# prs-eth/ResDepth

Hardware: AMD Instinct MI355X
Metric: DSM tiles/sec fwd+bwd (256x256, 3-ch, depth-5 U-Net) (higher is better)
Workload: dtype f32

## Files before the change

### resdepth_amd/csrc/rd_wgrad_strip.hip

```cpp
#include <stdlib.h>

#include "rd_common.h"
#include "rd_mfma_dev.h"

namespace rd {

struct WsParams {
    const float* dz;
    const float* x;
    float* slab;
    int Cin, Cout, M, N;
    int H, W;
    int strips_x, chunks_y, rows_per_chunk, reps;
    int tiles_ci, tiles_mn;
    unsigned a_bytes, b_bytes;
    const unsigned* a_amax;
    const unsigned* b_amax;
    int n_img;
};

typedef short v4s16 __attribute__((ext_vector_type(4)));
template <typename FR>
__device__ __forceinline__ FR lds_tr2(const float* smem_base, int byte_off, int second) {
    typedef __attribute__((address_space(3))) v4s16* lds_p;
    const char* b = reinterpret_cast<const char*>(smem_base) + byte_off;
    const v4s16 lo = __builtin_amdgcn_ds_read_tr16_b64_v4i16((lds_p)(b));
    const v4s16 hi = __builtin_amdgcn_ds_read_tr16_b64_v4i16((lds_p)(b + second));
    typedef short v8s16 __attribute__((ext_vector_type(8)));
    const v8s16 r = {lo.x, lo.y, lo.z, lo.w, hi.x, hi.y, hi.z, hi.w};
    return __builtin_bit_cast(FR, r);
}

template <int NP, int NCO, int NCI, bool W8>
__device__ __forceinline__ void wgrad_strip_tr_body(const WsParams& p, float* smem, const Quant qz) {
    typedef typename frag_of<NP>::type FR;
    constexpr int NT = NP == 3 ? 2 : 3;
    static_assert(NCO * NCI == 4, "four waves");
    constexpr int TA = 64 * NCO, TB = 64 * NCI;
    constexpr int APX = 3 * TA + (NCO == 4 ? 64 : NCO == 2 ? 64 : 0), BPX = 3 * TB + (NCI == 2 ? 64 : 0);
    static_assert((APX / 4) % 64 == 16 || (APX / 4) % 64 == 48, "dz pixel stride");
    static_assert((BPX / 4) % 64 == 16 || (BPX / 4) % 64 == 48, "x pixel stride");
    constexpr int HPX = W8 ? 20 : 18;
    constexpr int ASTAGE = 16 * APX, BSLOT = HPX * BPX;
    constexpr int RINGB = 2 * ASTAGE;
    constexpr int AQ = 8 * NCO, BQ = 8 * NCI;
    constexpr int AI = 16 * AQ / 256, BI = (HPX * BQ + 255) / 256;

    const int gb = xcd_remap(blockIdx.x, gridDim.x);
    const int split = gb / p.tiles_mn;
    const int lb = gb - split * p.tiles_mn;
    const int tile_ci = lb % p.tiles_ci, tile_m = lb / p.tiles_ci;
    const int m0 = tile_m * (32 * NCO), ci0 = tile_ci * (32 * NCI);
    int img = 0, x0 = 0, ya = 0, yb = 0;
    const int H = p.H, W = p.W;
    const int t = threadIdx.x, lane = t & 63, wave = t >> 6;
    const int cw = wave / NCI, cb = wave % NCI;

    int a_wr[AI], b_wr[BI];
    int a_px[AI], a_ch[AI], b_hp[BI], b_ch[BI];
    bool b_act[BI];
#pragma unroll
    for (int k = 0; k < AI; ++k) {
        const int e = t + 256 * k, cq = e % AQ, px = e / AQ;
        a_px[k] = px;
        a_ch[k] = m0 + cq * 4 < p.Cout ? m0 + cq * 4 : -1;
        a_wr[k] = px * APX + cq * 8;
    }
#pragma unroll
    for (int k = 0; k < BI; ++k) {
        const int e = t + 256 * k, cq = e % BQ, hp = e / BQ;
        b_act[k] = e < HPX * BQ;
        b_hp[k] = hp;
        b_ch[k] = (b_act[k] && ci0 + cq * 4 < p.Cin) ? ci0 + cq * 4 : -1;
        b_wr[k] = hp * BPX + cq * 8;
    }
    const __amdgpu_buffer_rsrc_t rsA = make_rsrc(p.dz, p.a_bytes), rsB = make_rsrc(p.x, p.b_bytes);
    const unsigned rowA = (unsigned)W * p.Cout * 4, rowB = (unsigned)W * p.Cin * 4;
    unsigned baseA = 0, baseB = 0, voffA[AI], voffB[BI];
    auto set_strip = [&](int sid) {
        const int sx = sid % p.strips_x;
        const int cy = (sid / p.strips_x) % p.chunks_y;
        img = sid / (p.strips_x * p.chunks_y);
        x0 = sx * 16;
        ya = cy * p.rows_per_chunk;
        yb = ya + p.rows_per_chunk;
        if (W8) img *= 2;
        baseA = (unsigned)img * H * rowA;
        baseB = (unsigned)img * H * rowB;
        if (W8) {
            const bool two = img + 1 < p.n_img;
#pragma unroll
            for (int k = 0; k < AI; ++k) {
                const int sub = a_px[k] >> 3, xx = a_px[k] & 7;
                voffA[k] = (a_ch[k] >= 0 && (sub == 0 || two)) ? (unsigned)(((sub * 64 + xx) * p.Cout + a_ch[k]) * 4) : kOOB;
            }
#pragma unroll
            for (int k = 0; k < BI; ++k) {
                const int sub = b_hp[k] >= 10 ? 1 : 0, px = b_hp[k] - 10 * sub - 1;
                voffB[k] = (b_ch[k] >= 0 && (unsigned)px < 8u && (sub == 0 || two)) ? (unsigned)(((sub * 64 + px) * p.Cin + b_ch[k]) * 4) : kOOB;
            }
            return;
        }
#pragma unroll
        for (int k = 0; k < AI; ++k) voffA[k] = a_ch[k] >= 0 ? (unsigned)(((x0 + a_px[k]) * p.Cout + a_ch[k]) * 4) : kOOB;
#pragma unroll
        for (int k = 0; k < BI; ++k) {
            const int px = x0 - 1 + b_hp[k];
            voffB[k] = (b_ch[k] >= 0 && (unsigned)px < (unsigned)W) ? (unsigned)((px * p.Cin + b_ch[k]) * 4) : kOOB;
        }
    };
    auto load_task = [&](int yy, float4 (&v)[AI + BI]) {
        const int ra = yy + 1, rb = yy + 2;
        const bool oka = ra >= ya && ra < yb, okb = rb >= 0 && rb < H && rb <= yb;
        const unsigned sa = (unsigned)__builtin_amdgcn_readfirstlane(oka ? (int)(baseA + (unsigned)ra * rowA) : 0);
        const unsigned sb = (unsigned)__builtin_amdgcn_readfirstlane(okb ? (int)(baseB + (unsigned)rb * rowB) : 0);
#pragma unroll
        for (int k = 0; k < AI; ++k) v[k] = buf_load4(rsA, oka ? voffA[k] : kOOB, sa);
#pragma unroll
        for (int k = 0; k < BI; ++k) v[AI + k] = buf_load4(rsB, okb ? voffB[k] : kOOB, sb);
    };
    auto put = [&](char* dst, int tstride, const float4 x, float qs) {
        uint2 ph, pm, pl;
        split_pack4v<NP, false>(x.x, x.y, x.z, x.w, qs, ph, pm, pl);
        *reinterpret_cast<uint2*>(dst) = ph;
        *reinterpret_cast<uint2*>(dst + tstride) = pm;
        if (kterm3<NP>()) *reinterpret_cast<uint2*>(dst + 2 * tstride) = pl;
    };
    auto store_task = [&](int yy, const float4 (&v)[AI + BI]) {
        char* sa = reinterpret_cast<char*>(smem) + ((yy + 1) & 1) * ASTAGE;
#pragma unroll
        for (int k = 0; k < AI; ++k) put(sa + a_wr[k], TA, v[k], qz.sa);
        char* sb = reinterpret_cast<char*>(smem) + RINGB + ((yy + 3) & 3) * BSLOT;
#pragma unroll
        for (int k = 0; k < BI; ++k)
            if (b_act[k]) put(sb + b_wr[k], TB, v[AI + k], qz.sb);
    };

    const int li = lane & 15, lg = lane >> 4, nb = lg & 1, hk = lg >> 1;
    const int a_rd = (8 * hk + (li >> 2)) * APX + (32 * cw + 16 * nb + 4 * (li & 3)) * 2;
    const int b_rd = (8 * hk + (li >> 2) + (W8 ? 2 * hk : 0)) * BPX + (32 * cb + 16 * nb + 4 * (li & 3)) * 2;
    const int lrow = lane & 31, half = lane >> 5;

    f32x16 acc[9];
#pragma unroll
    for (int tp = 0; tp < 9; ++tp)
#pragma unroll
        for (int r = 0; r < 16; ++r) acc[tp][r] = 0.f;

    constexpr int PA[6] = {2, 1, 0, 1, 0, 0}, PB[6] = {0, 1, 2, 0, 1, 0};
    auto mma_row = [&](int y) {
        const int a_stage = (y & 1) * ASTAGE;
        FR af[3], bf[2][3][3];
        auto read_b = [&](int dy, FR (&dst)[3][3]) {
            const int slot = RINGB + ((y + dy) & 3) * BSLOT;
#pragma unroll
            for (int d = 0; d < 3; ++d)
#pragma unroll
                for (int q = 0; q < NT; ++q) dst[d][q] = lds_tr2<FR>(smem, slot + b_rd + d * BPX + q * TB, 4 * BPX);
        };
#pragma unroll
        for (int q = 0; q < NT; ++q) af[q] = lds_tr2<FR>(smem, a_stage + a_rd + q * TA, 4 * APX);
        read_b(0, bf[0]);
#pragma unroll
        for (int dy = 0; dy < 3; ++dy) {
            if (dy < 2) read_b(dy + 1, bf[(dy + 1) & 1]);
#if RD_WG_FENCE
            if constexpr (NP == 3) __builtin_amdgcn_sched_barrier(0);
#endif
#pragma unroll
            for (int t6 = lo0<NP>(); t6 < 6; ++t6)
#pragma unroll
                for (int d = 0; d < 3; ++d) acc[dy * 3 + d] = mfma16<NP>(af[PA[t6]], bf[dy & 1][d][PB[t6]], acc[dy * 3 + d]);
        }
    };

    float4 v0[AI + BI], v1[AI + BI];
    for (int rep = 0; rep < p.reps; ++rep) {
        set_strip(split * p.reps + rep);
        const int ys = ya - 3;
        load_task(ys, v0);
        load_task(ys + 1, v1);
        store_task(ys, v0);
        load_task(ys + 2, v0);
        __syncthreads();
        store_task(ys + 1, v1);
        load_task(ys + 3, v1);
        __syncthreads();
        store_task(ys + 2, v0);
        load_task(ys + 4, v0);
        __syncthreads();
        for (int yy = ya; yy < yb; yy += 2) {
            store_task(yy, v1);
            load_task(yy + 2, v1);
            mma_row(yy);
            __syncthreads();
            store_task(yy + 1, v0);
            load_task(yy + 3, v0);
            mma_row(yy + 1);
            __syncthreads();
        }
    }

    float* out = p.slab + (long)split * p.M * p.N;
    const int cwu = __builtin_amdgcn_readfirstlane(cw), cbu = __builtin_amdgcn_readfirstlane(cb);
    if (m0 + 32 * NCO <= p.M && (long)(32 * NCO) * p.N * 4 < 0x7fffffffL) {
        const __amdgpu_buffer_rsrc_t rsO = make_rsrc(out + (long)m0 * p.N + ci0, (unsigned)((long)(32 * NCO) * p.N * 4));
        const unsigned lane_off = (unsigned)(((4 * half) * p.N + lrow) * 4);
        const int rowN = __builtin_amdgcn_readfirstlane(p.N * 4);
        const int base = (cwu * 32) * rowN + cbu * 128;
#pragma unroll
        for (int tp = 0; tp < 9; ++tp) {
            const int tapo = base + tp * p.Cin * 4;
#pragma unroll
            for (int r = 0; r < 16; ++r)
                __builtin_amdgcn_raw_buffer_store_b32(__float_as_int(scale_q<NP>(acc[tp][r], qz.dexp)), rsO, lane_off, (unsigned)(tapo + ((r & 3) + 8 * (r >> 2)) * rowN), 0);
        }
        return;
    }
#pragma unroll
    for (int tp = 0; tp < 9; ++tp) {
        const int n = tp * p.Cin + ci0 + cb * 32 + lrow;
#pragma unroll
        for (int r = 0; r < 16; ++r) {
            const int m = m0 + cw * 32 + (r & 3) + 8 * (r >> 2) + 4 * half;
            if (m < p.M) out[(long)m * p.N + n] = scale_q<NP>(acc[tp][r], qz.dexp);
        }
    }
}

template <int NCO, int NCI, bool W8>
__device__ __forceinline__ void wgrad_strip_rot_body(const WsParams& p, float* smem, const Quant qz) {
    typedef f16x8 FR;
    static_assert(NCO * NCI == 4, "four waves");
    constexpr int TA = 64 * NCO, TB = 64 * NCI;
    constexpr int APX = 3 * TA + (NCO == 4 ? 64 : NCO == 2 ? 64 : 0), BPX = 3 * TB + (NCI == 2 ? 64 : 0);
    constexpr int HPX = W8 ? 20 : 18;
    constexpr int ASTAGE = 16 * APX, BSLOT = HPX * BPX;
    constexpr int RINGB = 4 * ASTAGE;
    constexpr int AQ = 8 * NCO, BQ = 8 * NCI;
    constexpr int AI = 16 * AQ / 256, BI = (HPX * BQ + 255) / 256;

    const int gb = xcd_remap(blockIdx.x, gridDim.x);
    const int split = gb / p.tiles_mn;
    const int lb = gb - split * p.tiles_mn;
    const int tile_ci = lb % p.tiles_ci, tile_m = lb / p.tiles_ci;
    const int m0 = tile_m * (32 * NCO), ci0 = tile_ci * (32 * NCI);
    int img = 0, x0 = 0, ya = 0, yb = 0;
    const int H = p.H, W = p.W;
    const int t = threadIdx.x, lane = t & 63, wave = t >> 6;
    const int cw = wave / NCI, cb = wave % NCI;

    int a_wr[AI], b_wr[BI];
    int a_px[AI], a_ch[AI], b_hp[BI], b_ch[BI];
    bool b_act[BI];
#pragma unroll
    for (int k = 0; k < AI; ++k) {
        const int e = t + 256 * k, cq = e % AQ, px = e / AQ;
        a_px[k] = px;
        a_ch[k] = m0 + cq * 4 < p.Cout ? m0 + cq * 4 : -1;
        a_wr[k] = px * APX + cq * 8;
    }
#pragma unroll
    for (int k = 0; k < BI; ++k) {
        const int e = t + 256 * k, cq = e % BQ, hp = e / BQ;
        b_act[k] = e < HPX * BQ;
        b_hp[k] = hp;
        b_ch[k] = (b_act[k] && ci0 + cq * 4 < p.Cin) ? ci0 + cq * 4 : -1;
        b_wr[k] = hp * BPX + cq * 8;
    }
    const __amdgpu_buffer_rsrc_t rsA = make_rsrc(p.dz, p.a_bytes), rsB = make_rsrc(p.x, p.b_bytes);
    const unsigned rowA = (unsigned)W * p.Cout * 4, rowB = (unsigned)W * p.Cin * 4;
    unsigned baseA = 0, baseB = 0, voffA[AI], voffB[BI];
    auto set_strip = [&](int sid) {
        const int sx = sid % p.strips_x;
        const int cy = (sid / p.strips_x) % p.chunks_y;
        img = sid / (p.strips_x * p.chunks_y);
        x0 = sx * 16;
        ya = cy * p.rows_per_chunk;
        yb = ya + p.rows_per_chunk;
        if (W8) img *= 2;
        baseA = (unsigned)img * H * rowA;
        baseB = (unsigned)img * H * rowB;
        if (W8) {
            const bool two = img + 1 < p.n_img;
#pragma unroll
            for (int k = 0; k < AI; ++k) {
                const int sub = a_px[k] >> 3, xx = a_px[k] & 7;
                voffA[k] = (a_ch[k] >= 0 && (sub == 0 || two)) ? (unsigned)(((sub * 64 + xx) * p.Cout + a_ch[k]) * 4) : kOOB;
            }
#pragma unroll
            for (int k = 0; k < BI; ++k) {
                const int sub = b_hp[k] >= 10 ? 1 : 0, px = b_hp[k] - 10 * sub - 1;
                voffB[k] = (b_ch[k] >= 0 && (unsigned)px < 8u && (sub == 0 || two)) ? (unsigned)(((sub * 64 + px) * p.Cin + b_ch[k]) * 4) : kOOB;
            }
            return;
        }
#pragma unroll
        for (int k = 0; k < AI; ++k) voffA[k] = a_ch[k] >= 0 ? (unsigned)(((x0 + a_px[k]) * p.Cout + a_ch[k]) * 4) : kOOB;
#pragma unroll
        for (int k = 0; k < BI; ++k) {
            const int px = x0 - 1 + b_hp[k];
            voffB[k] = (b_ch[k] >= 0 && (unsigned)px < (unsigned)W) ? (unsigned)((px * p.Cin + b_ch[k]) * 4) : kOOB;
        }
    };
    auto load_task = [&](int k, float4 (&v)[AI + BI]) {
        const int r = k + 2;
        const bool oka = r >= ya && r < yb, okb = r >= 0 && r < H && r <= yb;
        const unsigned sa = (unsigned)__builtin_amdgcn_readfirstlane(oka ? (int)(baseA + (unsigned)r * rowA) : 0);
        const unsigned sb = (unsigned)__builtin_amdgcn_readfirstlane(okb ? (int)(baseB + (unsigned)r * rowB) : 0);
#pragma unroll
        for (int i = 0; i < AI; ++i) v[i] = buf_load4(rsA, oka ? voffA[i] : kOOB, sa);
#pragma unroll
        for (int i = 0; i < BI; ++i) v[AI + i] = buf_load4(rsB, okb ? voffB[i] : kOOB, sb);
    };
    auto put = [&](char* dst, int tstride, const float4 x, float qs) {
        uint2 ph, pm, pl;
        split_pack4v<3, false>(x.x, x.y, x.z, x.w, qs, ph, pm, pl);
        *reinterpret_cast<uint2*>(dst) = ph;
        *reinterpret_cast<uint2*>(dst + tstride) = pm;
    };
    auto store_task = [&](int k, const float4 (&v)[AI + BI]) {
        char* sa = reinterpret_cast<char*>(smem) + ((k + 2) & 3) * ASTAGE;
#pragma unroll
        for (int i = 0; i < AI; ++i) put(sa + a_wr[i], TA, v[i], qz.sa);
        char* sb = reinterpret_cast<char*>(smem) + RINGB + ((k + 2) & 1) * BSLOT;
#pragma unroll
        for (int i = 0; i < BI; ++i)
            if (b_act[i]) put(sb + b_wr[i], TB, v[AI + i], qz.sb);
    };

    const int li = lane & 15, lg = lane >> 4, nb = lg & 1, hk = lg >> 1;
    const int a_rd = (8 * hk + (li >> 2)) * APX + (32 * cw + 16 * nb + 4 * (li & 3)) * 2;
    const int b_rd = (8 * hk + (li >> 2) + (W8 ? 2 * hk : 0)) * BPX + (32 * cb + 16 * nb + 4 * (li & 3)) * 2;
    const int lrow = lane & 31, half = lane >> 5;

    f32x16 acc[9];
#pragma unroll
    for (int tp = 0; tp < 9; ++tp)
#pragma unroll
        for (int r = 0; r < 16; ++r) acc[tp][r] = 0.f;

    auto read_x = [&](int row, FR (&dst)[3][2]) {
        const int slot = RINGB + (row & 1) * BSLOT;
#pragma unroll
        for (int d = 0; d < 3; ++d)
#pragma unroll
            for (int q = 0; q < 2; ++q) dst[d][q] = lds_tr2<FR>(smem, slot + b_rd + d * BPX + q * TB, 4 * BPX);
    };
    auto read_dz = [&](int row, FR (&dst)[2]) {
        const int stage = (row & 3) * ASTAGE;
#pragma unroll
        for (int q = 0; q < 2; ++q) dst[q] = lds_tr2<FR>(smem, stage + a_rd + q * TA, 4 * APX);
    };
    auto group = [&](int dy, const FR (&af)[2], const FR (&xf)[3][2]) {
#pragma unroll
        for (int d = 0; d < 3; ++d) acc[dy * 3 + d] = mfma16<3>(af[1], xf[d][0], acc[dy * 3 + d]);
#pragma unroll
        for (int d = 0; d < 3; ++d) acc[dy * 3 + d] = mfma16<3>(af[0], xf[d][1], acc[dy * 3 + d]);
#pragma unroll
        for (int d = 0; d < 3; ++d) acc[dy * 3 + d] = mfma16<3>(af[0], xf[d][0], acc[dy * 3 + d]);
    };
    auto step = [&](int y, const FR (&af)[2], FR (&afn)[2], FR (&P)[3][2], const FR (&Q)[3][2]) {
        group(0, af, P);
        __builtin_amdgcn_sched_barrier(0);
        read_x(y + 1, P);
        read_dz(y + 1, afn);
        __builtin_amdgcn_sched_barrier(0);
        group(1, af, Q);
        __builtin_amdgcn_sched_barrier(0);
        group(2, af, P);
        __builtin_amdgcn_sched_barrier(0);
    };

    float4 v0[AI + BI], v1[AI + BI];
    FR xa[3][2], xb[3][2], af0[2], af1[2];
    for (int rep = 0; rep < p.reps; ++rep) {
        set_strip(split * p.reps + rep);
        load_task(ya - 3, v0);
        load_task(ya - 2, v1);
        store_task(ya - 3, v0);
        load_task(ya - 1, v0);
        store_task(ya - 2, v1);
        load_task(ya, v1);
        __syncthreads();
        read_x(ya - 1, xa);
        read_x(ya, xb);
        read_dz(ya, af0);
        __syncthreads();
        store_task(ya - 1, v0);
        load_task(ya + 1, v0);
        __syncthreads();
        for (int yy = ya; yy < yb; yy += 2) {
            store_task(yy, v1);
            load_task(yy + 2, v1);
            step(yy, af0, af1, xa, xb);
            __syncthreads();
            store_task(yy + 1, v0);
            load_task(yy + 3, v0);
            step(yy + 1, af1, af0, xb, xa);
            __syncthreads();
        }
    }

    float* out = p.slab + (long)split * p.M * p.N;
    const int cwu = __builtin_amdgcn_readfirstlane(cw), cbu = __builtin_amdgcn_readfirstlane(cb);
    if (m0 + 32 * NCO <= p.M && (long)(32 * NCO) * p.N * 4 < 0x7fffffffL) {
        const __amdgpu_buffer_rsrc_t rsO = make_rsrc(out + (long)m0 * p.N + ci0, (unsigned)((long)(32 * NCO) * p.N * 4));
        const unsigned lane_off = (unsigned)(((4 * half) * p.N + lrow) * 4);
        const int rowN = __builtin_amdgcn_readfirstlane(p.N * 4);
        const int base = (cwu * 32) * rowN + cbu * 128;
#pragma unroll
        for (int tp = 0; tp < 9; ++tp) {
            const int tapo = base + tp * p.Cin * 4;
#pragma unroll
            for (int r = 0; r < 16; ++r)
                __builtin_amdgcn_raw_buffer_store_b32(__float_as_int(scale_q<3>(acc[tp][r], qz.dexp)), rsO, lane_off, (unsigned)(tapo + ((r & 3) + 8 * (r >> 2)) * rowN), 0);
        }
        return;
    }
#pragma unroll
    for (int tp = 0; tp < 9; ++tp) {
        const int n = tp * p.Cin + ci0 + cb * 32 + lrow;
#pragma unroll
        for (int r = 0; r < 16; ++r) {
            const int m = m0 + cw * 32 + (r & 3) + 8 * (r >> 2) + 4 * half;
            if (m < p.M) out[(long)m * p.N + n] = scale_q<3>(acc[tp][r], qz.dexp);
        }
    }
}

template <int OCC, int NCO, int NCI, bool W8 = false>
__global__ __launch_bounds__(256, OCC) void wgrad_strip_tr_kernel(WsParams p) {
    constexpr int TA = 64 * NCO, TB = 64 * NCI;
    constexpr int APX = 3 * TA + (NCO == 4 ? 64 : NCO == 2 ? 64 : 0), BPX = 3 * TB + (NCI == 2 ? 64 : 0);
    constexpr int HPX = W8 ? 20 : 18, ASTAGE = 16 * APX, BSLOT = HPX * BPX;
    constexpr int SM6 = 2 * ASTAGE + 4 * BSLOT, SM3 = 4 * ASTAGE + 2 * BSLOT;
    __shared__ __attribute__((aligned(16))) float smem[(SM6 > SM3 ? SM6 : SM3) / 4];
    const Quant qz = quant_select(p.a_amax, p.b_amax);
#if RD_WG_NOROT
    if (qz.use3) wgrad_strip_tr_body<3, NCO, NCI, W8>(p, smem, qz);
#else
    if (qz.use3) wgrad_strip_rot_body<NCO, NCI, W8>(p, smem, qz);
#endif
    else wgrad_strip_tr_body<6, NCO, NCI, W8>(p, smem, qz);
}

struct WsPlan {
    int ok, swapped, rows_per_chunk, chunks_y, strips_x, tiles_m, tiles_ci, reps, splits;
    int sq;
    int w8;
};

static WsPlan plan_strip(int n, int h, int w, int cin, int cout) {
    WsPlan pl = {};
    const int force = tune(TUNE_WG_STRIP);
    const bool w8 = w == 8 && h == 8 && cout % 64 == 0 && cin % 64 == 0 && force != 1 && force != 3 && tune(TUNE_WG_STRIP) != 4;
    if (!mfma_split() || force == 0 || (!w8 && w % 16 != 0) || h < 4 || h % 2 != 0) return pl;
    if (force != 1 && force != 3 && cout % 64 == 0 && cin % 64 == 0) {
        pl.sq = 1;
    } else if (cout >= 128 && cout % 4 == 0 && cin % 32 == 0) {
        pl.swapped = 0;
    } else if (cin >= 128 && cin % 4 == 0 && cout % 32 == 0) {
        pl.swapped = 1;
        const int tmp = cin; cin = cout; cout = tmp;
    } else {
        return pl;
    }
    pl.ok = 1;
    pl.w8 = w8;
    if (w8) n = (n + 1) / 2;
    pl.strips_x = w8 ? 1 : w / 16;
    pl.tiles_m = cdiv(cout, pl.sq ? 64 : 128);
    pl.tiles_ci = cin / (pl.sq ? 64 : 32);
    const long base = (long)pl.tiles_m * pl.tiles_ci * n * pl.strips_x;
    int rows = h;
    const int minb = tune(TUNE_WG_MINBLOCKS);
    while (base * (h / rows) < minb && rows > 32 && rows % 4 == 0) rows >>= 1;
    pl.rows_per_chunk = rows;
    pl.chunks_y = h / rows;
    const long strips = (long)n * pl.strips_x * pl.chunks_y;
    const int target = tune(TUNE_WG_BLOCKS);
    int reps = 1;
    while (base * pl.chunks_y / (2 * reps) >= target && strips % (2 * reps) == 0) reps *= 2;
    pl.reps = reps;
    pl.splits = (int)(strips / reps);
    return pl;
}


int wgrad_strip_splits(int n, int h, int w, int cin, int cout) {
    const WsPlan pl = plan_strip(n, h, w, cin, cout);
    return pl.ok ? pl.splits : 0;
}

int wgrad_strip_launch(const float* x, const float* dz, float* slab, int n, int h, int w, int cin, int cout, hipStream_t s,
                       int* splits_out, int* swapped_out, const unsigned* x_amax, const unsigned* dz_amax) {
    const WsPlan wp = plan_strip(n, h, w, cin, cout);
    *splits_out = 0;
    *swapped_out = 0;
    if (!wp.ok) return RD_OK;
    if (wp.swapped) {
        const float* tp = x; x = dz; dz = tp;
        const int tc = cin; cin = cout; cout = tc;
        const unsigned* ta = x_amax; x_amax = dz_amax; dz_amax = ta;
    }
    WsParams q = {};
    q.dz = dz; q.x = x; q.slab = slab;
    q.Cin = cin; q.Cout = cout; q.M = cout; q.N = 9 * cin;
    q.H = h; q.W = w;
    q.strips_x = wp.strips_x; q.chunks_y = wp.chunks_y; q.rows_per_chunk = wp.rows_per_chunk; q.reps = wp.reps;
    q.tiles_ci = wp.tiles_ci; q.tiles_mn = wp.tiles_m * wp.tiles_ci;
    q.n_img = n;
    if (mfma_products() == 3 && x_amax && dz_amax) { q.a_amax = dz_amax; q.b_amax = x_amax; }
    const double ab = 4.0 * n * h * w * (double)cout, bb = 4.0 * n * h * w * (double)cin;
    RD_REQUIRE(ab < 4294967040.0 && bb < 4294967040.0, "rd_conv3x3_bwd_weight: operand beyond the 4 GiB descriptor range");
    q.a_bytes = (unsigned)ab; q.b_bytes = (unsigned)bb;
    const int occ_ = tune(TUNE_WG_OCC) == 2 ? 2 : 1;
    char pcls[64];
    if (wp.w8) snprintf(pcls, sizeof(pcls), "conv3x3_wgrad|wgrad_strip_tr<%d,2,2,w8>", occ_);
    else if (wp.sq) snprintf(pcls, sizeof(pcls), "conv3x3_wgrad|wgrad_strip_tr<%d,2,2>", occ_);
    else snprintf(pcls, sizeof(pcls), "conv3x3_wgrad|wgrad_strip_tr<%d,4,1>", occ_);
    ProfScope ps(s, pcls, 2.0 * cout * 9.0 * cin * (double)n * h * w, ab + bb + 4.0 * cout * 9.0 * cin, true);
    const dim3 grid(q.tiles_mn * wp.splits);
    const int occ = tune(TUNE_WG_OCC);
    if (wp.w8 && occ == 2) RD_LAUNCH((wgrad_strip_tr_kernel<2, 2, 2, true>), grid, dim3(256), 0, s, q);
    else if (wp.w8) RD_LAUNCH((wgrad_strip_tr_kernel<1, 2, 2, true>), grid, dim3(256), 0, s, q);
    else if (wp.sq && occ == 2) RD_LAUNCH((wgrad_strip_tr_kernel<2, 2, 2>), grid, dim3(256), 0, s, q);
    else if (wp.sq) RD_LAUNCH((wgrad_strip_tr_kernel<1, 2, 2>), grid, dim3(256), 0, s, q);
    else if (occ == 2) RD_LAUNCH((wgrad_strip_tr_kernel<2, 4, 1>), grid, dim3(256), 0, s, q);
    else RD_LAUNCH((wgrad_strip_tr_kernel<1, 4, 1>), grid, dim3(256), 0, s, q);
    RD_LAUNCH_CHECK("wgrad_strip");
    *splits_out = wp.splits;
    *swapped_out = wp.swapped;
    return RD_OK;
}

}
```

Measured before the change: 4589.

## Interleave wgrad staging loads and f16 splits between individual MFMAs

Breaks each per-row staging task (global buffer load, two-way f16 hi/lo split, LDS store) into small pieces and schedules one piece behind each of the first eighteen MFMAs of a step, fenced with sched_barrier, instead of doing the whole store/load batch before the MMA groups. It also adds inline-asm v_fma_mix helpers that produce the hi and residual halves directly, and a tune-selected fallback ring kernel that keeps the old path. The goal is to hide VALU, VMEM and LDS-write latency under matrix-core work. The price is rigid instruction ordering and more live registers, which could raise register pressure.

```diff
diff --git a/resdepth_amd/csrc/rd_wgrad_strip.hip b/resdepth_amd/csrc/rd_wgrad_strip.hip
--- a/resdepth_amd/csrc/rd_wgrad_strip.hip
+++ b/resdepth_amd/csrc/rd_wgrad_strip.hip
@@ -228,6 +228,18 @@
     }
 }
 
+__device__ __forceinline__ unsigned split2h_hi(float x0, float x1, float s) {
+    unsigned ph;
+    asm("v_fma_mixlo_f16 %0, %1, %3, 0\n\tv_fma_mixhi_f16 %0, %2, %3, 0" : "=&v"(ph) : "v"(x0), "v"(x1), "s"(s));
+    return ph;
+}
+__device__ __forceinline__ unsigned split2h_lo(float x0, float x1, float s, unsigned ph) {
+    unsigned pm;
+    asm("v_fma_mixlo_f16 %0, %1, %3, -%4 op_sel_hi:[0,0,1]\n\tv_fma_mixhi_f16 %0, %2, %3, -%4 op_sel:[0,0,1] op_sel_hi:[0,0,1]"
+        : "=&v"(pm)
+        : "v"(x0), "v"(x1), "s"(s), "v"(ph));
+    return pm;
+}
 template <int NCO, int NCI, bool W8>
 __device__ __forceinline__ void wgrad_strip_rot_body(const WsParams& p, float* smem, const Quant qz) {
     typedef f16x8 FR;
@@ -239,6 +251,8 @@
     constexpr int RINGB = 4 * ASTAGE;
     constexpr int AQ = 8 * NCO, BQ = 8 * NCI;
     constexpr int AI = 16 * AQ / 256, BI = (HPX * BQ + 255) / 256;
+    constexpr int NI = AI + BI;
+    static_assert(6 * NI <= 18, "six staging pieces per item, one behind each of a step's first eighteen MFMAs");
 
     const int gb = xcd_remap(blockIdx.x, gridDim.x);
     const int split = gb / p.tiles_mn;
@@ -263,7 +277,7 @@
 #pragma unroll
     for (int k = 0; k < BI; ++k) {
         const int e = t + 256 * k, cq = e % BQ, hp = e / BQ;
-        b_act[k] = e < HPX * BQ;
+        b_act[k] = 256 * k + 255 < HPX * BQ || e < HPX * BQ;
         b_hp[k] = hp;
         b_ch[k] = (b_act[k] && ci0 + cq * 4 < p.Cin) ? ci0 + cq * 4 : -1;
         b_wr[k] = hp * BPX + cq * 8;
@@ -303,30 +317,52 @@
             voffB[k] = (b_ch[k] >= 0 && (unsigned)px < (unsigned)W) ? (unsigned)((px * p.Cin + b_ch[k]) * 4) : kOOB;
         }
     };
-    auto load_task = [&](int k, float4 (&v)[AI + BI]) {
+    auto load_item = [&](int k, int i, float4 (&v)[NI]) {
         const int r = k + 2;
-        const bool oka = r >= ya && r < yb, okb = r >= 0 && r < H && r <= yb;
-        const unsigned sa = (unsigned)__builtin_amdgcn_readfirstlane(oka ? (int)(baseA + (unsigned)r * rowA) : 0);
-        const unsigned sb = (unsigned)__builtin_amdgcn_readfirstlane(okb ? (int)(baseB + (unsigned)r * rowB) : 0);
-#pragma unroll
-        for (int i = 0; i < AI; ++i) v[i] = buf_load4(rsA, oka ? voffA[i] : kOOB, sa);
-#pragma unroll
-        for (int i = 0; i < BI; ++i) v[AI + i] = buf_load4(rsB, okb ? voffB[i] : kOOB, sb);
-    };
-    auto put = [&](char* dst, int tstride, const float4 x, float qs) {
-        uint2 ph, pm, pl;
-        split_pack4v<3, false>(x.x, x.y, x.z, x.w, qs, ph, pm, pl);
-        *reinterpret_cast<uint2*>(dst) = ph;
-        *reinterpret_cast<uint2*>(dst + tstride) = pm;
-    };
-    auto store_task = [&](int k, const float4 (&v)[AI + BI]) {
-        char* sa = reinterpret_cast<char*>(smem) + ((k + 2) & 3) * ASTAGE;
-#pragma unroll
-        for (int i = 0; i < AI; ++i) put(sa + a_wr[i], TA, v[i], qz.sa);
-        char* sb = reinterpret_cast<char*>(smem) + RINGB + ((k + 2) & 1) * BSLOT;
-#pragma unroll
-        for (int i = 0; i < BI; ++i)
-            if (b_act[i]) put(sb + b_wr[i], TB, v[AI + i], qz.sb);
+        if (i < AI) {
+            const bool oka = r >= ya && r < yb;
+            const unsigned sa = (unsigned)__builtin_amdgcn_readfirstlane(oka ? (int)(baseA + (unsigned)r * rowA) : 0);
+            v[i] = buf_load4(rsA, oka ? voffA[i] : kOOB, sa);
+        } else {
+            const bool okb = r >= 0 && r < H && r <= yb;
+            const unsigned sb = (unsigned)__builtin_amdgcn_readfirstlane(okb ? (int)(baseB + (unsigned)r * rowB) : 0);
+            v[i] = buf_load4(rsB, okb ? voffB[i - AI] : kOOB, sb);
+        }
+    };
+    auto split_piece = [&](int k, int i, int piece, const float4 (&v)[NI], uint2& ph, uint2& pm) {
+        const float qs = i < AI ? qz.sa : qz.sb;
+        if (piece == 0) ph.x = split2h_hi(v[i].x, v[i].y, qs);
+        else if (piece == 1) ph.y = split2h_hi(v[i].z, v[i].w, qs);
+        else if (piece == 2) pm.x = split2h_lo(v[i].x, v[i].y, qs, ph.x);
+        else if (piece == 3) pm.y = split2h_lo(v[i].z, v[i].w, qs, ph.y);
+        else {
+            char* dst = reinterpret_cast<char*>(smem) +
+                        (i < AI ? ((k + 2) & 3) * ASTAGE + a_wr[i] : RINGB + ((k + 2) & 1) * BSLOT + b_wr[i - AI]);
+            *reinterpret_cast<uint2*>(dst) = ph;
+            *reinterpret_cast<uint2*>(dst + (i < AI ? TA : TB)) = pm;
+        }
+    };
+    auto stage_piece = [&](int k, int i, int piece, float4 (&v)[NI], uint2& ph, uint2& pm) {
+        const bool whole = i < AI || 256 * (i - AI) + 255 < HPX * BQ;
+        if (piece == 5) load_item(k + 2, i, v);
+        else if (whole) split_piece(k, i, piece, v, ph, pm);
+        else if (piece == 0) {
+            if (b_act[i - AI]) {
+#pragma unroll
+                for (int q = 0; q < 5; ++q) split_piece(k, i, q, v, ph, pm);
+            }
+        }
+    };
+    auto load_task = [&](int k, float4 (&v)[NI]) {
+#pragma unroll
+        for (int i = 0; i < NI; ++i) load_item(k, i, v);
+    };
+    auto store_task = [&](int k, float4 (&v)[NI]) {
+        uint2 ph, pm;
+#pragma unroll
+        for (int i = 0; i < NI; ++i)
+#pragma unroll
+            for (int piece = 0; piece < 5; ++piece) stage_piece(k, i, piece, v, ph, pm);
     };
 
     const int li = lane & 15, lg = lane >> 4, nb = lg & 1, hk = lg >> 1;
@@ -360,19 +396,28 @@
 #pragma unroll
         for (int d = 0; d < 3; ++d) acc[dy * 3 + d] = mfma16<3>(af[0], xf[d][0], acc[dy * 3 + d]);
     };
-    auto step = [&](int y, const FR (&af)[2], FR (&afn)[2], FR (&P)[3][2], const FR (&Q)[3][2]) {
-        group(0, af, P);
+    auto mma_staged = [&](int dy, int m, const FR (&af)[2], const FR (&xf)[3][2], int y, int j, float4 (&v)[NI], uint2& ph, uint2& pm) {
+        const int d = m % 3;
+        acc[dy * 3 + d] = mfma16<3>(af[m < 3 ? 1 : 0], xf[d][m >= 3 && m < 6 ? 1 : 0], acc[dy * 3 + d]);
         __builtin_amdgcn_sched_barrier(0);
+        if (j < 6 * NI) stage_piece(y, j / 6, j % 6, v, ph, pm);
+        __builtin_amdgcn_sched_barrier(0);
+    };
+    auto step = [&](int y, float4 (&v)[NI], const FR (&af)[2], FR (&afn)[2], FR (&P)[3][2], const FR (&Q)[3][2]) {
+        uint2 ph, pm;
+        __builtin_amdgcn_sched_barrier(0);
+#pragma unroll
+        for (int m = 0; m < 9; ++m) mma_staged(0, m, af, P, y, m, v, ph, pm);
         read_x(y + 1, P);
         read_dz(y + 1, afn);
         __builtin_amdgcn_sched_barrier(0);
-        group(1, af, Q);
-        __builtin_amdgcn_sched_barrier(0);
+#pragma unroll
+        for (int m = 0; m < 9; ++m) mma_staged(1, m, af, Q, y, 9 + m, v, ph, pm);
         group(2, af, P);
         __builtin_amdgcn_sched_barrier(0);
     };
 
-    float4 v0[AI + BI], v1[AI + BI];
+    float4 v0[NI], v1[NI];
     FR xa[3][2], xb[3][2], af0[2], af1[2];
     for (int rep = 0; rep < p.reps; ++rep) {
         set_strip(split * p.reps + rep);
@@ -391,13 +436,9 @@
         load_task(ya + 1, v0);
         __syncthreads();
         for (int yy = ya; yy < yb; yy += 2) {
-            store_task(yy, v1);
-            load_task(yy + 2, v1);
-            step(yy, af0, af1, xa, xb);
+            step(yy, v1, af0, af1, xa, xb);
             __syncthreads();
-            store_task(yy + 1, v0);
-            load_task(yy + 3, v0);
-            step(yy + 1, af1, af0, xb, xa);
+            step(yy + 1, v0, af1, af0, xb, xa);
             __syncthreads();
         }
     }
@@ -429,19 +470,28 @@
     }
 }
 
+template <int NCO, int NCI, bool W8>
+struct WsSmem {
+    static constexpr int TA = 64 * NCO, TB = 64 * NCI;
+    static constexpr int APX = 3 * TA + (NCO == 4 ? 64 : NCO == 2 ? 64 : 0), BPX = 3 * TB + (NCI == 2 ? 64 : 0);
+    static constexpr int HPX = W8 ? 20 : 18, ASTAGE = 16 * APX, BSLOT = HPX * BPX;
+    static constexpr int SM6 = 2 * ASTAGE + 4 * BSLOT, SM3 = 4 * ASTAGE + 2 * BSLOT;
+    static constexpr int FLOATS = (SM6 > SM3 ? SM6 : SM3) / 4;
+};
+
 template <int OCC, int NCO, int NCI, bool W8 = false>
 __global__ __launch_bounds__(256, OCC) void wgrad_strip_tr_kernel(WsParams p) {
-    constexpr int TA = 64 * NCO, TB = 64 * NCI;
-    constexpr int APX = 3 * TA + (NCO == 4 ? 64 : NCO == 2 ? 64 : 0), BPX = 3 * TB + (NCI == 2 ? 64 : 0);
-    constexpr int HPX = W8 ? 20 : 18, ASTAGE = 16 * APX, BSLOT = HPX * BPX;
-    constexpr int SM6 = 2 * ASTAGE + 4 * BSLOT, SM3 = 4 * ASTAGE + 2 * BSLOT;
-    __shared__ __attribute__((aligned(16))) float smem[(SM6 > SM3 ? SM6 : SM3) / 4];
+    __shared__ __attribute__((aligned(16))) float smem[WsSmem<NCO, NCI, W8>::FLOATS];
     const Quant qz = quant_select(p.a_amax, p.b_amax);
-#if RD_WG_NOROT
+    if (qz.use3) wgrad_strip_rot_body<NCO, NCI, W8>(p, smem, qz);
+    else wgrad_strip_tr_body<6, NCO, NCI, W8>(p, smem, qz);
+}
+
+template <int NCO, int NCI, bool W8 = false>
+__global__ __launch_bounds__(256, 1) void wgrad_strip_ring_kernel(WsParams p) {
+    __shared__ __attribute__((aligned(16))) float smem[WsSmem<NCO, NCI, W8>::FLOATS];
+    const Quant qz = quant_select(p.a_amax, p.b_amax);
     if (qz.use3) wgrad_strip_tr_body<3, NCO, NCI, W8>(p, smem, qz);
-#else
-    if (qz.use3) wgrad_strip_rot_body<NCO, NCI, W8>(p, smem, qz);
-#endif
     else wgrad_strip_tr_body<6, NCO, NCI, W8>(p, smem, qz);
 }
 
@@ -523,7 +573,11 @@
     ProfScope ps(s, pcls, 2.0 * cout * 9.0 * cin * (double)n * h * w, ab + bb + 4.0 * cout * 9.0 * cin, true);
     const dim3 grid(q.tiles_mn * wp.splits);
     const int occ = tune(TUNE_WG_OCC);
-    if (wp.w8 && occ == 2) RD_LAUNCH((wgrad_strip_tr_kernel<2, 2, 2, true>), grid, dim3(256), 0, s, q);
+    if (tune(TUNE_WG_STRIP) == 5) {
+        if (wp.w8) RD_LAUNCH((wgrad_strip_ring_kernel<2, 2, true>), grid, dim3(256), 0, s, q);
+        else if (wp.sq) RD_LAUNCH((wgrad_strip_ring_kernel<2, 2>), grid, dim3(256), 0, s, q);
+        else RD_LAUNCH((wgrad_strip_ring_kernel<4, 1>), grid, dim3(256), 0, s, q);
+    } else if (wp.w8 && occ == 2) RD_LAUNCH((wgrad_strip_tr_kernel<2, 2, 2, true>), grid, dim3(256), 0, s, q);
     else if (wp.w8) RD_LAUNCH((wgrad_strip_tr_kernel<1, 2, 2, true>), grid, dim3(256), 0, s, q);
     else if (wp.sq && occ == 2) RD_LAUNCH((wgrad_strip_tr_kernel<2, 2, 2>), grid, dim3(256), 0, s, q);
     else if (wp.sq) RD_LAUNCH((wgrad_strip_tr_kernel<1, 2, 2>), grid, dim3(256), 0, s, q);
```

Result: no change. 4631 (median of 6 runs) (+0.9%).
